# abelxiaoxing/ImageClassification

Measured on AMD Instinct MI355X. Metric: images/sec (whole node) ResNet-50 bf16 224^2 training, higher is better.
Workload: dtype bf16; 1 GPU; resnet50 train step, synthetic 3x224x224, batch 256/GPU, AdamW, label smoothing 0.1, 1000 classes (BASELINE configs[1]); global_batch=256, parallelism=dp1

## Files before the change

imageclassification_amd/csrc/capi.hip:

```cpp
#include "../../include/icamd.h"
#include "common.h"
#include "icamd_internal.h"
#include <cstdlib>
#include <string.h>

int icamd_bn_finalize_launch(const float* part, int nrows, int C, double count, const float* gamma, const float* beta,
                             float* running_mean, float* running_var, float momentum, float eps, float* mean,
                             float* invstd, float* scale, float* shift, double* chunks, hipStream_t s);
int icamd_bn_eval_coeffs_launch(int C, const float* gamma, const float* beta, const float* rm, const float* rv, float eps,
                                float* scale, float* shift, hipStream_t s);
int icamd_bn_apply_launch(const bf16_t* y, const float* scale, const float* shift, const bf16_t* residual, bf16_t* out,
                          unsigned char* maskbits, long long numel, int C, int relu, hipStream_t s,
                          const float* res_scale = nullptr, const float* res_shift = nullptr);
int icamd_bn_bwd_rows_per_block(long long rows, int C);
int icamd_bn_bwd_launch(const bf16_t* dout, const bf16_t* act, const bf16_t* y, const float* mean, const float* invstd,
                        const float* scale, const float* shift, float* dgamma, float* dbeta, bf16_t* dy, bf16_t* gout,
                        const unsigned char* maskbits, long long rows, int C, int relu, int accumulate, float* part,
                        double* chunks, float* c1c2, hipStream_t s, const unsigned char* pool_idx = nullptr,
                        int pool_ih = 0, int pool_iw = 0);
int icamd_bn_bwd_dual_launch(const bf16_t* dout, const unsigned char* maskbits, const bf16_t* yA, const float* meanA,
                             const float* invstdA, const float* scaleA, float* dgammaA, float* dbetaA, bf16_t* dyA,
                             const bf16_t* yB, const float* meanB, const float* invstdB, const float* scaleB, float* dgammaB,
                             float* dbetaB, bf16_t* dyB, long long rows, int C, int accumulate, float* partA, double* chunksA,
                             float* cA, float* partB, double* chunksB, float* cB, hipStream_t s);
// ... 115 lines not shown
  return c;
}
}

namespace {

bool conv_desc_ok(const icamd_conv_desc* d) {
  if (d == nullptr) return false;
  if (d->N <= 0 || d->IH <= 0 || d->IW <= 0 || d->Cin <= 0 || d->OH <= 0 || d->OW <= 0 || d->Cout <= 0) return false;
  if (d->KH <= 0 || d->KW <= 0 || d->stride <= 0 || d->pad < 0) return false;
  if (d->Cin % 64 == 0 && d->KH * d->KW > ICAMD_MAX_TAPS) return false;
  if (d->KH * d->KW > 1024) return false;
  if ((d->IH + 2 * d->pad - d->KH) / d->stride + 1 != d->OH) return false;
  if ((d->IW + 2 * d->pad - d->KW) / d->stride + 1 != d->OW) return false;
  return true;
}

inline size_t align_up(size_t v, size_t a) { return (v + a - 1) / a * a; }

}

extern "C" {

int icamd_abi_version(void) { return 5; }

int icamd_prof_enable(int on) { g_prof_on = on != 0; return ICAMD_OK; }
int icamd_prof_classes(void) { return PC_COUNT; }
int icamd_prof_collect(double* ms, long long* calls, double* bytes, double* flops, int n) {
  if (ms == nullptr || calls == nullptr || n < PC_COUNT) return ICAMD_ERR_BAD_ARG;
  for (auto& r : g_prof_recs) {
    (void)hipEventSynchronize(r.b);
    float t = 0.f;
    (void)hipEventElapsedTime(&t, r.a, r.b);
    ms[r.cls] += (double)t;
    calls[r.cls] += 1;
    if (bytes != nullptr) bytes[r.cls] += r.bytes;
    if (flops != nullptr) flops[r.cls] += r.flops;
    g_prof_pool.push_back(r.a);
    g_prof_pool.push_back(r.b);
  }
  g_prof_recs.clear();
  return ICAMD_OK;
}

int icamd_conv2d_stats_rows(const icamd_conv_desc* d) {
  if (!conv_desc_ok(d)) return 0;
  const long long M = (long long)d->N * d->OH * d->OW;
// ... 218 lines not shown
  return dgrad_impl(d, dy, w_t, dz, nullptr, nullptr, nullptr, stream, z);
}

int icamd_conv2d_dgrad_stats_rows(const icamd_conv_desc* d) {
  if (!conv_desc_ok(d)) return 0;
  int rows = 0;
  for (int ph = 0; ph < d->stride; ++ph)
    for (int pw = 0; pw < d->stride; ++pw) {
      const long long P = (d->IH - ph + d->stride - 1) / d->stride, Q = (d->IW - pw + d->stride - 1) / d->stride;
      if (P > 0 && Q > 0) rows += (int)((d->N * P * Q + 127) / 128);
    }
  return rows;
}

int icamd_conv2d_dgrad_bnbwd(const icamd_conv_desc* d, const void* dy, const void* w_t, void* g, const void* addend,
                             const icamd_bn_bwd_fuse* f, void* stream) {
  ProfScope _prof(PC_IGEMM_DGRAD, stream);
  const ConvWork cw = conv_work(d); _prof.work(cw.out + 2 * cw.in + 2 * cw.w + (addend ? cw.in : 0), cw.flops);
  if (f == nullptr || f->y == nullptr || f->mean == nullptr || f->invstd == nullptr || f->partials == nullptr)
    return ICAMD_ERR_BAD_ARG;
  return dgrad_impl(d, dy, w_t, g, addend, nullptr, f, stream);
}

int icamd_conv2d_dgrad_bnred_supported(const icamd_conv_desc* d) {
  if (!conv_desc_ok(d) || d->KH != 1 || d->KW != 1 || d->stride != 1 || d->pad != 0) return 0;
  return icamd_pw_resident_bnred_wanted((long long)d->N * d->IH * d->IW, d->Cin, d->Cout) ? 1 : 0;
}

int icamd_conv2d_dgrad_bnred(const icamd_conv_desc* d, const void* dy, const void* w_t, void* g, const void* addend,
                             const uint8_t* addend_bits, int addend_sub2, const void* bn_y, const uint8_t* bn_bits,
                             float* partials, void* stream) {
  ProfScope _prof(PC_IGEMM_DGRAD, stream);
  const ConvWork cw = conv_work(d); _prof.work(cw.out + 3 * cw.in + 2 * cw.w + cw.in / 16 + (addend_bits ? cw.in / 16 : 0), cw.flops);
  if (!conv_desc_ok(d) || dy == nullptr || w_t == nullptr || g == nullptr || addend == nullptr || bn_y == nullptr ||
      bn_bits == nullptr || partials == nullptr || (addend_sub2 && addend_bits != nullptr))
    return ICAMD_ERR_BAD_ARG;
  if (!icamd_conv2d_dgrad_bnred_supported(d)) return ICAMD_ERR_UNSUPPORTED;
  PwResidentParams p;
  memset(&p, 0, sizeof(p));
  p.A = (const bf16_t*)dy; p.B = (const bf16_t*)w_t; p.out = (bf16_t*)g; p.addend = (const bf16_t*)addend;
  p.addend_bits = addend_bits;
  p.bn_y = (const bf16_t*)bn_y; p.bn_bits = bn_bits; p.bn_part = partials;
  p.M = d->N * d->IH * d->IW; p.N = d->Cin; p.K = d->Cout;
  if (addend_sub2) { p.sub2_h = d->IH; p.sub2_w = d->IW; }
  return icamd_pw_resident_bnred_launch(p, (hipStream_t)stream);
}
// ... 189 lines not shown
  if (dout == nullptr || maskbits == nullptr || yA == nullptr || yB == nullptr || meanA == nullptr || meanB == nullptr ||
      invstdA == nullptr || invstdB == nullptr || scaleA == nullptr || scaleB == nullptr || dgammaA == nullptr ||
      dgammaB == nullptr || dbetaA == nullptr || dbetaB == nullptr || dyA == nullptr || dyB == nullptr ||
      workspaceA == nullptr || workspaceB == nullptr || workspaceA == workspaceB || rows <= 0 || C <= 0)
    return ICAMD_ERR_BAD_ARG;
  if (workspace_bytes < icamd_bn_bwd_workspace_bytes(rows, C)) return ICAMD_ERR_WORKSPACE;
  if (C > 4096) return ICAMD_ERR_UNSUPPORTED;
  const int rpb = icamd_bn_bwd_rows_per_block(rows, C);
  const long long nblk = (rows + rpb - 1) / rpb;
  float* part[2]; double* chunks[2]; float* cc[2];
  void* wsv[2] = {workspaceA, workspaceB};
  for (int i = 0; i < 2; ++i) {
    char* ws = (char*)wsv[i];
    chunks[i] = (double*)(ws + 256);
    ws += bn_chunk_bytes(C);
    part[i] = (float*)ws;
    ws += align_up((size_t)nblk * 2 * C * sizeof(float), 256);
    cc[i] = (float*)ws;
  }
  return icamd_bn_bwd_dual_launch((const bf16_t*)dout, maskbits, (const bf16_t*)yA, meanA, invstdA, scaleA, dgammaA, dbetaA,
                                  (bf16_t*)dyA, (const bf16_t*)yB, meanB, invstdB, scaleB, dgammaB, dbetaB, (bf16_t*)dyB, rows,
                                  C, accumulate, part[0], chunks[0], cc[0], part[1], chunks[1], cc[1], (hipStream_t)stream);
}

size_t icamd_bn_bwd_apply_workspace_bytes(int C) {
  return C > 0 ? bn_chunk_bytes(C) + align_up((size_t)2 * C * sizeof(float), 256) : 0;
}

int icamd_bn_bwd_from_partials(const float* partials, int nrows, const void* g, const void* y, const float* mean,
                               const float* invstd, const float* scale, float* dgamma, float* dbeta, void* dy,
                               long long rows, int C, int accumulate, void* workspace, size_t workspace_bytes,
                               void* stream) {
  ProfScope _prof(PC_BN_BWD, stream);
  _prof.work((double)rows * C * 6 + 8.0 * nrows * C);
  if (partials == nullptr || nrows <= 0 || g == nullptr || y == nullptr || mean == nullptr || invstd == nullptr ||
      scale == nullptr || dgamma == nullptr || dbeta == nullptr || dy == nullptr || workspace == nullptr || rows <= 0 ||
      C <= 0 || C % 8 != 0)
    return ICAMD_ERR_BAD_ARG;
  if (workspace_bytes < icamd_bn_bwd_apply_workspace_bytes(C)) return ICAMD_ERR_WORKSPACE;
  if (C > 4096) return ICAMD_ERR_UNSUPPORTED;
  char* ws = (char*)workspace;
  double* chunks = (double*)(ws + 256);
  ws += bn_chunk_bytes(C);
  return icamd_bn_bwd_apply_launch(partials, nrows, (const bf16_t*)g, (const bf16_t*)y, mean, invstd, scale, dgamma, dbeta,
                                   (bf16_t*)dy, rows, C, accumulate, chunks, (float*)ws, (hipStream_t)stream);
}
// ... 579 lines not shown
```

imageclassification_amd/csrc/conv3x3_halo.hip:

```cpp
#ifndef ICAMD_C64_NT
#define ICAMD_C64_NT 0
#endif
#include "common.h"
#include "icamd_internal.h"
#include <cstdlib>

namespace {

template <int N> __device__ __forceinline__ void halo_wait_vmcnt() {
  static_assert(N >= 0 && N < 64, "vmcnt is a 6-bit field");
  asm volatile("s_waitcnt vmcnt(%0)" ::"n"(N) : "memory");
}

__device__ __forceinline__ int swzq(int blk) { return (0x78 >> (2 * blk)) & 3; }

template <int BN, int WN, int MFR, int LA, int NB, int KS, int WPS>
__global__ __launch_bounds__(256, WPS) void conv3x3_halo_kernel(const Halo3x3Params p) {
  constexpr int WM = 4 / WN;
  constexpr int BM = WM * MFR * 16;
  constexpr int NJ = BN / WN / 16;
  constexpr int A_SLOTS = 4 * LA * 8;
  constexpr int ZERO_SLOT = A_SLOTS - 1;
  constexpr int A_BYTES = A_SLOTS * 128;
  constexpr int B_STAGE = BN * KS * 2;
// ... 215 lines not shown
  if (p.stats != nullptr) {
    __syncthreads();
    float* red = (float*)smem;
#pragma unroll
    for (int e = 0; e < 8; ++e) {
      red[(rg * 2 + 0) * BN + cp * 8 + e] = s1[e];
      red[(rg * 2 + 1) * BN + cp * 8 + e] = s2[e];
    }
    __syncthreads();
    const int ntm = (p.M + BM - 1) / BM, nrows = (p.M + 127) / 128;
    for (int idx = tid; idx < 2 * BN; idx += 256) {
      const int which = idx / BN, c = idx - which * BN;
      float s = 0.f;
#pragma unroll 4
      for (int g = 0; g < RPP; ++g) s += red[(g * 2 + which) * BN + c];
      if (n0 + c < p.Cout) {
        p.stats[((long long)tile_m * 2 + which) * p.Cout + n0 + c] = s;
        if (ntm + tile_m < nrows) p.stats[((long long)(ntm + tile_m) * 2 + which) * p.Cout + n0 + c] = 0.f;
      }
    }
  }
}

template <bool ACT>
__global__ __launch_bounds__(256, 2) void conv3x3_c64_resident_kernel(const Halo3x3Params p, const int ntiles) {
  constexpr int BM = 128, LA = 8;
  constexpr int A_BYTES = 32 * LA * 128;
  constexpr int E_BYTES = 4 * 64 * 64;
  constexpr int ZERO_SLOT = 32 * LA - 1;
  __shared__ __attribute__((aligned(16))) unsigned char smem[2 * A_BYTES + E_BYTES];

  const int tid = threadIdx.x, lane = tid & 63;
  const int wave = __builtin_amdgcn_readfirstlane(tid >> 6);
  const int wm = wave & 1, wn = wave >> 1;
  const int fr = lane & 15, fq = lane >> 4;
  const int W = p.W, H = p.H;
  const bf16_t* __restrict__ in = p.in;
  const bf16_t* zero = (const bf16_t*)icamd_zero_page;
  unsigned char* const sE = smem + 2 * A_BYTES + wave * 4096;
  const unsigned lds_base = (unsigned)(uintptr_t)LPTR(smem);

  const int a_slot = wave * 8 + (lane >> 3);
  const int a_lc = (((lane & 7) - (lane >> 3)) & 7) * 8;
  const bool a_zero_lane = a_slot == 31;
  auto stage_a = [&](int m0, unsigned char* dst) {
    const int pix0 = m0 - (W + 1) + a_slot;
    const bf16_t* src0 = in + ((long long)pix0 * 64 + a_lc);
// ... 112 lines not shown
    for (int j = 0; j < 2; ++j) {
      f32x4 b4 = {0.f, 0.f, 0.f, 0.f};
      if constexpr (ACT) {
        if (p.bias != nullptr) b4 = *(const f32x4*)(p.bias + wn * 32 + j * 16 + 4 * fq);
      }
#pragma unroll
      for (int i = 0; i < 4; ++i) {
        const int pl = i * 16 + fr;
        f32x4 v = acc[j][i];
        if constexpr (ACT) {
          v += b4;
          if (p.relu) {
#pragma unroll
            for (int e = 0; e < 4; ++e) v[e] = v[e] < 0.f ? 0.f : v[e];
          }
        }
        u32x2 pk;
        pk[0] = pack_bf16x2(v[0], v[1]);
        pk[1] = pack_bf16x2(v[2], v[3]);
        const int slot = j * 4 + fq;
        *(u32x2*)(sE + pl * 64 + ((((slot >> 1) ^ (pl >> 2)) & 3) << 4) + ((slot & 1) << 3)) = pk;
      }
    }
    {
      const int pl0 = lane >> 2;
      const int mrow = m0 + wm * 64 + pl0;
      bf16_t* orow = p.out + ((long long)mrow * 64 + wn * 32 + (lane & 3) * 8);
      const bool want_stats = p.stats != nullptr;
#pragma unroll
      for (int r = 0; r < 4; ++r) {
        const int pl = r * 16 + pl0;
        const u32x4 o = *(const u32x4*)(sE + pl * 64 + ((((lane & 3) ^ (pl >> 2)) & 3) << 4));
        if (mrow + r * 16 < p.M) {
          *(u32x4*)(orow + r * (16 * 64)) = o;
          if (want_stats) {
#pragma unroll
            for (int e = 0; e < 4; ++e) {
              const f32x2 v = {bf16_lo(o[e]), bf16_hi(o[e])};
              s1[e] += v;
              s2[e] = __builtin_elementwise_fma(v, v, s2[e]);
            }
          }
        }
      }
    }
  }

  if (p.stats != nullptr) {
    __syncthreads();
    float* red = (float*)smem;
    const int g = wm * 16 + (lane >> 2);
    const int c0 = wn * 32 + (lane & 3) * 8;
#pragma unroll
    for (int e = 0; e < 4; ++e) {
      red[(g * 2 + 0) * 64 + c0 + 2 * e] = s1[e][0];
      red[(g * 2 + 0) * 64 + c0 + 2 * e + 1] = s1[e][1];
      red[(g * 2 + 1) * 64 + c0 + 2 * e] = s2[e][0];
      red[(g * 2 + 1) * 64 + c0 + 2 * e + 1] = s2[e][1];
    }
    __syncthreads();
    if (tid < 128) {
      const int which = tid >> 6, c = tid & 63;
      float s = 0.f;
#pragma unroll 8
      for (int k = 0; k < 32; ++k) s += red[(k * 2 + which) * 64 + c];
      p.stats[((long long)blockIdx.x * 2 + which) * 64 + c] = s;
      const int nrows = (p.M + 127) / 128;
      for (int r = blockIdx.x + gridDim.x; r < nrows; r += gridDim.x) p.stats[((long long)r * 2 + which) * 64 + c] = 0.f;
    }
  }
}

int launch_resident_c64(const Halo3x3Params& p, hipStream_t stream) {
  const int ntiles = (p.M + 127) / 128;
  const int slots = 2 * icamd_num_cus();
  const int grid = ntiles < slots ? ntiles : slots;
  if (p.bias != nullptr || p.relu)
    hipLaunchKernelGGL((conv3x3_c64_resident_kernel<true>), dim3((unsigned)grid), dim3(256), 0, stream, p, ntiles);
  else
    hipLaunchKernelGGL((conv3x3_c64_resident_kernel<false>), dim3((unsigned)grid), dim3(256), 0, stream, p, ntiles);
  return icamd_launch_status();
}

template <int BN, int WN, int MFR, int LA, int NB, int KS, int WPS>
int launch_halo(const Halo3x3Params& p, hipStream_t stream) {
  constexpr int BM = (4 / WN) * MFR * 16;
  const int ntm = (p.M + BM - 1) / BM;
  hipLaunchKernelGGL((conv3x3_halo_kernel<BN, WN, MFR, LA, NB, KS, WPS>), dim3((unsigned)(ntm * p.ntiles_n)), dim3(256), 0,
                     stream, p);
  return icamd_launch_status();
}

int halo_mode() {
  static const int m = [] { const char* e = getenv("ICAMD_CONV3X3_HALO"); return e ? atoi(e) : 1; }();
  return m;
}

}

static bool resident_c64_ok(int W, int C, int Cout) {
  static const int on = [] { const char* e = getenv("ICAMD_CONV3X3_RESIDENT"); return e ? atoi(e) : 1; }();
  return on != 0 && C == 64 && Cout == 64 && W % 8 == 0 && 128 + 2 * W + 2 <= 255;
}

bool icamd_halo3x3_wanted(int N, int H, int W, int C, int Cout) {
  if (halo_mode() == 0) return false;
  if (C % 64 != 0 || Cout % 8 != 0 || W < 3 || H < 3) return false;
  if (resident_c64_ok(W, C, Cout)) return true;
  if (halo_mode() == 1 && C < 256) return false;
  if ((long long)N * H * W >= (1ll << 30)) return false;
  if (2 * W + 3 + 128 > 4 * 8 * 8) return false;
  return true;
}

int icamd_halo3x3_launch(Halo3x3Params& p, hipStream_t stream) {
  if (!icamd_halo3x3_wanted(p.N, p.H, p.W, p.C, p.Cout)) return ICAMD_ERR_UNSUPPORTED;
  p.M = p.N * p.H * p.W;
  p.divHW = make_fastdiv((unsigned)(p.H * p.W));
  p.divW = make_fastdiv((unsigned)p.W);
  if (resident_c64_ok(p.W, p.C, p.Cout)) return launch_resident_c64(p, stream);
  const int bn = p.Cout <= 64 ? 64 : 128;
  p.ntiles_n = (p.Cout + bn - 1) / bn;
  int bm = 128;
  if (halo_mode() == 3) bm = 256;
  else if (halo_mode() != 2) {
    long long best = -1;
    for (int cand : {256, 224, 128}) {
      if (cand == 224 && bn != 128) continue;
      if ((cand + 2 * p.W + 3 + 31) / 32 > (cand == 128 ? 8 : 12)) continue;
      const long long tiles = (long long)((p.M + cand - 1) / cand) * p.ntiles_n;
      const long long cost = ((tiles + 511) / 512) * cand + (cand == 128 ? 16 : 0);
      if (best < 0 || cost < best) { best = cost; bm = cand; }
    }
  }
  const bool big = bm != 128;
  const int slots = bm + 2 * p.W + 2 + 1;
  const int la = (slots + 31) / 32;
  if (la > 12) return ICAMD_ERR_UNSUPPORTED;
  if (bn == 128) {
// ... 24 lines not shown
```

imageclassification_amd/csrc/icamd_internal.h:

```cpp
#pragma once
#include "common.h"

#define ICAMD_MAX_TAPS 56

struct IgemmParams {
  const bf16_t* in;
  const bf16_t* wt;
  bf16_t* out;
  const bf16_t* addend;
  const unsigned char* addend_bits;
  int addend_sub2;
  const float* bias;
  float* stats;
  const bf16_t* bnb_y;
  const bf16_t* bnb_mask;
  const float *bnb_mean, *bnb_invstd, *bnb_scale, *bnb_shift;
  int bnb_relu;
  int relu;
  bf16_t* gelu_out;
  int gelu_inplace;
  const bf16_t* gelu_z;
  int N, IH, IW, Cin;
  int OH, OW, Cout;
  int P, Q, M;
  int ostr, ooff_h, ooff_w, istr;
  int ntaps, Ktot;
  int KW, pad;
  int tap_sign, regular_taps;
  int stem7;
  int ksteps, ntiles_n;
  FastDiv divPQ, divQ, divCin, divKW;
  short dh[ICAMD_MAX_TAPS], dw[ICAMD_MAX_TAPS], wtap[ICAMD_MAX_TAPS];
};
int icamd_igemm_launch(IgemmParams& p, hipStream_t stream);
int icamd_igemm_pick_bn(int Cout);

struct Halo3x3Params {
  const bf16_t* in;
  const bf16_t* wt;
  bf16_t* out;
  const float* bias;
  float* stats;
  int relu;
  int flip;
  int N, H, W, C, Cout;
  int M, ntiles_n;
  FastDiv divHW, divW;
};
bool icamd_halo3x3_wanted(int N, int H, int W, int C, int Cout);
int icamd_halo3x3_launch(Halo3x3Params& p, hipStream_t stream);

struct GemmNtParams {
  const bf16_t* A;
  const bf16_t* B;
  bf16_t* out;
  const bf16_t* addend;
  const unsigned char* addend_bits;
  const float* bias;
  float* stats;
  int M, N, K;
  int sub2_h, sub2_w;
  FastDiv divHW, divW;
  int relu;
  bf16_t* gelu_out;
  int gelu_inplace;
  const bf16_t* gelu_z;
  int ntiles_n;
  int group_n;
  int out_policy;
};
int icamd_gemm_nt_launch(GemmNtParams& p, hipStream_t stream);
bool icamd_gemm_nt_wanted(long long M, int N, int K);
// ... 108 lines not shown
```

imageclassification_amd/hip.py:

```python
import ctypes
import os
from ctypes import POINTER, Structure, c_double, c_float, c_int, c_longlong, c_size_t, c_void_p

import torch

_HERE = os.path.dirname(os.path.abspath(__file__))
LIB_PATH = os.path.join(_HERE, "csrc", "libicamd.so")

ABI_VERSION = 5
ERRORS = {1: "ICAMD_ERR_BAD_ARG", 2: "ICAMD_ERR_UNSUPPORTED", 3: "ICAMD_ERR_WORKSPACE", 4: "ICAMD_ERR_LAUNCH"}


class IcamdError(RuntimeError):
    pass


class BnBwdFuse(Structure):
    _fields_ = [("y", c_void_p), ("mask_src", c_void_p), ("mean", c_void_p), ("invstd", c_void_p), ("scale", c_void_p),
                ("shift", c_void_p), ("partials", c_void_p), ("relu", c_int)]


class ImageDesc(Structure):
    _fields_ = [("src_offset", ctypes.c_int64), ("src_h", c_int), ("src_w", c_int), ("crop_top", c_int), ("crop_left", c_int),
                ("crop_h", c_int), ("crop_w", c_int), ("hflip", c_int), ("vflip", c_int), ("jitter_order", c_int * 3),
                ("jitter_factor", c_float * 3), ("erase_top", c_int), ("erase_left", c_int), ("erase_h", c_int),
                ("erase_w", c_int), ("erase_seed", ctypes.c_uint32), ("reserved", c_int)]


class ConvDesc(Structure):
    _fields_ = [(n, c_int) for n in ("N", "IH", "IW", "Cin", "OH", "OW", "Cout", "KH", "KW", "stride", "pad")]

    def key(self):
        return tuple(getattr(self, n) for n, _ in self._fields_)


def conv_desc(N, IH, IW, Cin, Cout, KH, KW, stride, pad):
    OH = (IH + 2 * pad - KH) // stride + 1
    OW = (IW + 2 * pad - KW) // stride + 1
    return ConvDesc(N, IH, IW, Cin, OH, OW, Cout, KH, KW, stride, pad)


_P = c_void_p
_SIGNATURES = {
    "icamd_abi_version": (c_int, []),
    "icamd_conv2d_fwd_gelu": (c_int, [_P, _P, _P, _P, _P, _P, _P]),
    "icamd_conv2d_dgrad_gelu": (c_int, [_P, _P, _P, _P, _P, _P]),
    "icamd_conv2d_fwd_act": (c_int, [_P, _P, _P, _P, _P, _P, c_int, _P]),
    "icamd_bn_fold_filters": (c_int, [_P, _P, _P, _P, _P, c_float, c_int, c_int, _P, _P, _P]),
    "icamd_conv2d_stats_rows": (c_int, [POINTER(ConvDesc)]),
    "icamd_conv2d_fwd": (c_int, [POINTER(ConvDesc), _P, _P, _P, _P, _P, _P, _P]),
    "icamd_conv2d_dgrad": (c_int, [POINTER(ConvDesc), _P, _P, _P, _P, _P, _P]),
    "icamd_conv2d_dgrad_sub2": (c_int, [POINTER(ConvDesc), _P, _P, _P, _P, _P]),
    "icamd_conv2d_dgrad_stats_rows": (c_int, [POINTER(ConvDesc)]),
    "icamd_conv2d_dgrad_bnbwd": (c_int, [POINTER(ConvDesc), _P, _P, _P, _P, POINTER(BnBwdFuse), _P]),
    "icamd_conv2d_dgrad_bnred_supported": (c_int, [POINTER(ConvDesc)]),
    "icamd_conv2d_dgrad_bnred": (c_int, [POINTER(ConvDesc), _P, _P, _P, _P, _P, c_int, _P, _P, _P, _P]),
    "icamd_bn_bwd_from_gy_partials": (c_int, [_P, c_int, _P, _P, _P, _P, _P, _P, _P, _P, c_longlong, c_int, c_int, _P, c_size_t, _P]),
    "icamd_bn_apply_conv1x1_fused_supported": (c_int, [POINTER(ConvDesc)]),
    "icamd_bn_apply_conv1x1_fused": (c_int, [POINTER(ConvDesc), _P, _P, _P, _P, _P, _P, _P, _P, _P, _P, _P, _P]),
    "icamd_conv1x1_bn_bwd_fused_supported": (c_int, [POINTER(ConvDesc)]),
    "icamd_conv1x1_bn_bwd_fused_workspace_bytes": (c_size_t, [POINTER(ConvDesc)]),
    "icamd_conv1x1_bn_bwd_fused": (c_int, [POINTER(ConvDesc), _P, c_int, _P, _P, _P, _P, _P, _P, _P, _P, _P, _P, _P, c_int, _P, c_size_t,
                                           _P, c_size_t, _P]),
    "icamd_conv2d_wgrad_workspace_bytes": (c_size_t, [POINTER(ConvDesc)]),
    "icamd_conv2d_wgrad": (c_int, [POINTER(ConvDesc), _P, _P, _P, c_int, _P, c_size_t, _P]),
    "icamd_conv2d_wgrad_bias": (c_int, [POINTER(ConvDesc), _P, _P, _P, _P, c_int, _P, c_size_t, _P]),
    "icamd_filter_transpose": (c_int, [_P, _P, _P, _P, c_int, _P]),
    "icamd_filter_transpose_tiled": (c_int, [_P, _P, _P, _P, c_int, _P]),
    "icamd_bn_workspace_bytes": (c_size_t, [c_int]),
    "icamd_bn_train_finalize": (c_int, [_P, c_int, c_int, c_double, _P, _P, _P, _P, c_float, c_float, _P, _P, _P, _P, _P, _P]),
    "icamd_bn_eval_coeffs": (c_int, [c_int, _P, _P, _P, _P, c_float, _P, _P, _P]),
    "icamd_bn_apply": (c_int, [_P, _P, _P, _P, _P, _P, c_longlong, c_int, c_int, _P]),
    "icamd_bn_apply_res_bn": (c_int, [_P, _P, _P, _P, _P, _P, _P, _P, c_longlong, c_int, c_int, _P]),
    "icamd_bn_bwd_workspace_bytes": (c_size_t, [c_longlong, c_int]),
    "icamd_bn_bwd": (c_int, [_P, _P, _P, _P, _P, _P, _P, _P, _P, _P, _P, _P, c_longlong, c_int, c_int, c_int, _P, c_size_t, _P]),
    "icamd_bn_bwd_maxpool3x3s2": (c_int, [_P, _P, _P, _P, _P, _P, _P, _P, _P, _P, c_int, c_int, c_int, c_int, c_int, _P, c_size_t, _P]),
    "icamd_bn_bwd_dual": (c_int, [_P, _P, _P, _P, _P, _P, _P, _P, _P, _P, _P, _P, _P, _P, _P, _P, c_longlong, c_int, c_int,
# ... 128 lines not shown
```

imageclassification_amd/nets.py:

```python
import ctypes
import math
import os
from collections import OrderedDict

import torch

from . import hip
from .checkpoint import PicklableModel

BN_EPS = 1e-5
_FUSED_BNBWD = os.environ.get("ICAMD_FUSED_BNBWD", "0") == "1"
_WGRAD_STREAM = os.environ.get("ICAMD_WGRAD_STREAM", "1") != "0"
_DUAL_BNBWD = os.environ.get("ICAMD_DUAL_BNBWD", "1") != "0"
_SUB2_SHORTCUT = os.environ.get("ICAMD_SUB2_SHORTCUT", "1") != "0"
_FUSED_POOL_BWD = os.environ.get("ICAMD_FUSED_POOL_BWD", "0") == "1"
BN_MOMENTUM = 0.1

ARCHS = {
    "resnet18": ("basic", [2, 2, 2, 2]),
    "resnet34": ("basic", [3, 4, 6, 3]),
    "resnet50": ("bottleneck", [3, 4, 6, 3]),
}


def _align(n, a):
    return (n + a - 1) // a * a


class _Param:
    __slots__ = ("name", "offset", "numel", "torch_shape", "kind", "padded_shape")

    def __init__(self, name, offset, numel, torch_shape, kind, padded_shape):
        self.name, self.offset, self.numel = name, offset, numel
        self.torch_shape, self.kind, self.padded_shape = torch_shape, kind, padded_shape


class _Conv:
# ... 372 lines not shown
            return ws
        dev = self.device
        lib = self.lib
        ws = {"N": N, "H": H, "W": W}

        def act(n, h, w, c):
            return torch.empty(n, h, w, c, dtype=torch.bfloat16, device=dev)

        Ws = W + (W & 1)
        ws["Ws"] = Ws
        ws["x8"] = act(N, H, Ws + 8, 4)
        d0 = self.stem_conv.desc(N, H, Ws)
        ws["y0"] = act(N, d0.OH, d0.OW, 64)
        ws["a0"] = act(N, d0.OH, d0.OW, 64)
        PH, PW = (d0.OH - 1) // 2 + 1, (d0.OW - 1) // 2 + 1
        ws["p0"] = act(N, PH, PW, 64)
        ws["p0_idx"] = torch.empty(N, PH, PW, 64, dtype=torch.uint8, device=dev)
        max_act = max(ws["y0"].numel(), ws["x8"].numel())
        max_stats = lib.icamd_conv2d_stats_rows(ctypes.byref(d0)) * 2 * 64
        max_wg = lib.icamd_stem7x7s2_wgrad_workspace_bytes(N, H, Ws, 64)
        max_bnb = lib.icamd_bn_bwd_workspace_bytes(N * d0.OH * d0.OW, 64)
        h, w = PH, PW
        blocks_ws = []
        for blk in self.blocks:
            b = {}
            ih, iw = h, w
            ys, acts = [], []
            for ci, conv in enumerate(blk["convs"]):
                d = conv.desc(N, ih, iw)
                ys.append(act(N, d.OH, d.OW, conv.cout_p))
                acts.append(act(N, d.OH, d.OW, conv.cout_p))
                max_act = max(max_act, ys[-1].numel())
                max_stats = max(max_stats, lib.icamd_conv2d_stats_rows(ctypes.byref(d)) * 2 * conv.cout_p)
                max_wg = max(max_wg, lib.icamd_conv2d_wgrad_workspace_bytes(ctypes.byref(d)))
                max_bnb = max(max_bnb, lib.icamd_bn_bwd_workspace_bytes(N * d.OH * d.OW, conv.cout_p))
                ih, iw = d.OH, d.OW
            b["y"], b["a"] = ys, acts
            b["mask"] = torch.empty(acts[-1].numel() // 8, dtype=torch.uint8, device=dev)
            if "down_conv" in blk:
                dd = blk["down_conv"].desc(N, h, w)
                b["yd"] = act(N, dd.OH, dd.OW, blk["down_conv"].cout_p)
                b["ad"] = act(N, dd.OH, dd.OW, blk["down_conv"].cout_p)
                max_stats = max(max_stats, lib.icamd_conv2d_stats_rows(ctypes.byref(dd)) * 2 * blk["down_conv"].cout_p)
                max_wg = max(max_wg, lib.icamd_conv2d_wgrad_workspace_bytes(ctypes.byref(dd)))
                max_bnb = max(max_bnb, lib.icamd_bn_bwd_workspace_bytes(N * dd.OH * dd.OW, blk["down_conv"].cout_p))
            blocks_ws.append(b)
            h, w = ih, iw
        ws["blocks"] = blocks_ws
        ws["final_hw"] = (h, w)
        ws["pooled"] = torch.empty(N, self.feat_dim, dtype=torch.bfloat16, device=dev)
        ws["logits"] = torch.zeros(N, self.ncls_p, dtype=torch.bfloat16, device=dev)
        dfc = self.fc.desc(N, 1, 1)
        max_wg = max(max_wg, lib.icamd_conv2d_wgrad_workspace_bytes(ctypes.byref(dfc)))
        ws["stats"] = torch.empty(max_stats, dtype=torch.float32, device=dev)
        ws["bn_ws"] = torch.zeros(lib.icamd_bn_workspace_bytes(2048), dtype=torch.uint8, device=dev)
        ws["wgrad_ws"] = torch.empty(max_wg, dtype=torch.uint8, device=dev)
        ws["wgrad_ws_bytes"] = max_wg
        ws["bnb_part"] = torch.empty(max_stats + 4 * 2 * 2048, dtype=torch.float32, device=dev)
        ws["bna_ws_bytes"] = lib.icamd_bn_bwd_apply_workspace_bytes(2048)
        ws["bna_ws"] = torch.zeros(ws["bna_ws_bytes"], dtype=torch.uint8, device=dev)
        ws["bnb_ws"] = torch.zeros(max_bnb, dtype=torch.uint8, device=dev)
        ws["bnb_ws2"] = torch.zeros(max_bnb, dtype=torch.uint8, device=dev)
        ws["bnb_ws_bytes"] = max_bnb
        ws["max_act"] = max_act
        ws["loss_rows"] = torch.empty(N, dtype=torch.float32, device=dev)
        ws["pred"] = torch.empty(N, dtype=torch.int32, device=dev)
        ws["dlogits"] = torch.zeros(N, self.ncls_p, dtype=torch.bfloat16, device=dev)
        ws["dpooled"] = torch.empty(N, self.feat_dim, dtype=torch.bfloat16, device=dev)
        ws["scale_shift_eval"] = torch.empty(2 * 2048, dtype=torch.float32, device=dev)
        self._ws[key] = ws
        return ws

    def _grad_buffers(self, ws):
        if "gbuf" not in ws:
            n = ws["max_act"]
            ws["gbuf"] = [torch.empty(n, dtype=torch.bfloat16, device=self.device) for _ in range(8)]
        return ws["gbuf"]

    def _w(self, conv):
        return self.shadow.data_ptr() + 2 * conv.w.offset

# ... 208 lines not shown

        dl = ws["dlogits"].data_ptr()
        wgrad(self.fc, ws["pooled"].data_ptr(), dl, N, 1, 1)
        hip.check(lib.icamd_colsum(dl, N, self.ncls_p, self.ncls_p, self._gf(self.fc.b), acc, s), "fc bias grad")
        dgrad(self.fc, dl, ws["dpooled"].data_ptr(), None, N, 1, 1)
        if hook:
            hook(self.fc.w.offset, self.n_params, side_events())
        fh, fw = ws["final_hw"]
        dout, other = D0, D1
        hip.check(lib.icamd_avgpool_bwd(ws["dpooled"].data_ptr(), dout, N, fh * fw, self.feat_dim, s), "avgpool bwd")

        fused_rows = 0
        for bi in range(len(self.blocks) - 1, -1, -1):
            blk, b = self.blocks[bi], ws["blocks"][bi]
            convs, bns = blk["convs"], blk["bns"]
            h, w = b["in_hw"]
            xin = b["in"]
            nconv = len(convs)
            hw_in = [(h, w)]
            for conv in convs[:-1]:
                d = conv.desc(N, *hw_in[-1])
                hw_in.append((d.OH, d.OW))
            mask = b["mask"].data_ptr()
            yk = next_y()
            y2 = None
            fused_conv3 = False
            shortcut_done = False
            prev_takes_g = False
            if bi > 0 and self.block == "bottleneck":
                pblk = self.blocks[bi - 1]
                if "down_conv" not in pblk:
                    prev_takes_g = True
                else:
                    dp3 = pblk["convs"][-1].desc(N, h, w)
                    prev_takes_g = bool(lib.icamd_conv1x1_bn_bwd_fused_supported(ctypes.byref(dp3)))
            d3 = convs[-1].desc(N, *hw_in[-1])
            fuse3 = (self.block == "bottleneck" and fused_rows > 0
                     and bool(lib.icamd_conv1x1_bn_bwd_fused_supported(ctypes.byref(d3))))

            def fused_conv_bn(conv, bn, dsc, partials, nrows, y_t, x_ptr, dx_ptr, bn_ws, bn_ws_bytes):
                st_ = self.stat_arena.data_ptr() + 4 * bn.stat_offset
                c_ = bn.c
                need = lib.icamd_conv1x1_bn_bwd_fused_workspace_bytes(ctypes.byref(dsc))
                fws = ws.get("fused_ws")
                if fws is None or fws.numel() < need:
                    fws = ws["fused_ws"] = torch.empty(need, dtype=torch.uint8, device=self.device)
                hip.check(lib.icamd_conv1x1_bn_bwd_fused(ctypes.byref(dsc), partials, nrows, dout, y_t.data_ptr(), st_, st_ + 4 * c_,
                                                         st_ + 8 * c_, self._gf(bn.weight), self._gf(bn.bias), x_ptr, self._wt(conv),
                                                         dx_ptr, self._gf(conv.w), acc, bn_ws, bn_ws_bytes, fws.data_ptr(),
                                                         fws.numel(), s), bn.name + " + " + conv.name + " bwd (fused)")

            if "down_conv" in blk and fuse3:
                fused_conv_bn(convs[-1], bns[-1], d3, ws["bnb_part"].data_ptr(), fused_rows, b["y"][-1],
                              b["a"][nconv - 2].data_ptr(), DA, ws["bna_ws"].data_ptr(), ws["bna_ws_bytes"])
                fused_conv3 = True
                dc = blk["down_conv"]
                ddc = dc.desc(N, h, w)
                if dc.stride == 1 and lib.icamd_conv1x1_bn_bwd_fused_supported(ctypes.byref(ddc)):
                    fused_conv_bn(dc, blk["down_bn"], ddc, None, 0, b["yd"], xin.data_ptr(), T, bws, bwb)
                    shortcut_done = True
                else:
                    y2 = next_y()
                    bn_bwd(blk["down_bn"], dout, None, b["yd"], ypool[y2], None, False)
            elif "down_conv" in blk and _DUAL_BNBWD:
                y2 = next_y()
                bnA, bnB = bns[-1], blk["down_bn"]
                stA = self.stat_arena.data_ptr() + 4 * bnA.stat_offset
                stB = self.stat_arena.data_ptr() + 4 * bnB.stat_offset
                c = bnA.c
                hip.check(lib.icamd_bn_bwd_dual(dout, mask, b["y"][-1].data_ptr(), stA, stA + 4 * c, stA + 8 * c,
                                                self._gf(bnA.weight), self._gf(bnA.bias), ypool[yk], b["yd"].data_ptr(), stB,
                                                stB + 4 * c, stB + 8 * c, self._gf(bnB.weight), self._gf(bnB.bias), ypool[y2],
                                                b["y"][-1].numel() // c, c, acc, bws, ws["bnb_ws2"].data_ptr(), bwb, s),
                          bnA.name + " + shortcut bwd")
            elif fused_rows:
                bnl = bns[-1]
                stl = self.stat_arena.data_ptr() + 4 * bnl.stat_offset
                cl = bnl.c
                if fuse3:
                    fused_conv_bn(convs[-1], bnl, d3, ws["bnb_part"].data_ptr(), fused_rows, b["y"][-1],
                                  b["a"][nconv - 2].data_ptr(), DA, ws["bna_ws"].data_ptr(), ws["bna_ws_bytes"])
                    fused_conv3 = True
                else:
                    hip.check(lib.icamd_bn_bwd_from_gy_partials(ws["bnb_part"].data_ptr(), fused_rows, dout, b["y"][-1].data_ptr(),
                                                                stl, stl + 4 * cl, stl + 8 * cl, self._gf(bnl.weight),
                                                                self._gf(bnl.bias), ypool[yk], b["y"][-1].numel() // cl, cl, acc,
                                                                ws["bna_ws"].data_ptr(), ws["bna_ws_bytes"], s),
                              bnl.name + " bwd (apply, sums from the data gradient)")
            else:
                bn_bwd(bns[-1], dout, None, b["y"][-1], ypool[yk], None, True, mask)
            fused_rows = 0
            for i in range(nconv - 1, 0, -1):
                x_i = b["a"][i - 1]
                if fused_conv3 and i == nconv - 1:
                    yk = next_y()
                    bn_bwd(bns[i - 1], DA, None, b["y"][i - 1], ypool[yk], None, True)
                    continue
                wgrad(convs[i], x_i.data_ptr(), ypool[yk], N, *hw_in[i], ybuf=yk)
                dgrad(convs[i], ypool[yk], DA, None, N, *hw_in[i])
                yk = next_y()
                bn_bwd(bns[i - 1], DA, None, b["y"][i - 1], ypool[yk], None, True)
            wgrad(convs[0], xin.data_ptr(), ypool[yk], N, h, w, ybuf=yk)
            if shortcut_done:
                dgrad(convs[0], ypool[yk], other, T, N, h, w)
            elif "down_conv" in blk:
                if y2 is None:
                    y2 = next_y()
                    bn_bwd(blk["down_bn"], dout, None, b["yd"], ypool[y2], None, True, mask)
                dc = blk["down_conv"]
                wgrad(dc, xin.data_ptr(), ypool[y2], N, h, w, ybuf=y2)
                if _SUB2_SHORTCUT and dc.k == 1 and dc.stride == 2 and dc.pad == 0:
                    dd = dc.desc(N, h, w)
                    key = ("sub2", N, dd.OH, dd.OW)
                    d1 = dc.descs.get(key)
                    if d1 is None:
                        d1 = dc.descs[key] = hip.conv_desc(N, dd.OH, dd.OW, dc.cin_p, dc.cout_p, 1, 1, 1, 0)
                    hip.check(lib.icamd_conv2d_dgrad(ctypes.byref(d1), ypool[y2], self._wt(dc), T, None, None, s),
                              dc.name + " dgrad (even grid)")
                    d0 = convs[0].desc(N, h, w)
                    if (prev_takes_g and self.block == "bottleneck"
                            and lib.icamd_conv2d_dgrad_bnred_supported(ctypes.byref(d0))):
# ... 160 lines not shown
```

include/icamd.h:

```cpp
#ifndef ICAMD_H
#define ICAMD_H
#include <stddef.h>
#include <stdint.h>

#ifdef __cplusplus
extern "C" {
#endif

#define ICAMD_OK 0
#define ICAMD_ERR_BAD_ARG 1
#define ICAMD_ERR_UNSUPPORTED 2
#define ICAMD_ERR_WORKSPACE 3
#define ICAMD_ERR_LAUNCH 4

int icamd_abi_version(void);

typedef struct icamd_conv_desc {
  int N, IH, IW, Cin;
  int OH, OW, Cout;
  int KH, KW, stride, pad;
} icamd_conv_desc;

int icamd_conv2d_stats_rows(const icamd_conv_desc* d);

// ... 53 lines not shown
                 const float* scale, const float* shift, float* dgamma, float* dbeta, void* dy, void* gout,
                 const uint8_t* maskbits, long long rows, int C, int relu, int accumulate, void* workspace,
                 size_t workspace_bytes, void* stream);
int icamd_bn_bwd_maxpool3x3s2(const void* dout_pooled, const uint8_t* idx, const void* y, const float* mean,
                              const float* invstd, const float* scale, const float* shift, float* dgamma, float* dbeta,
                              void* dy, int N, int IH, int IW, int C, int accumulate, void* workspace, size_t workspace_bytes,
                              void* stream);

int icamd_bn_bwd_dual(const void* dout, const uint8_t* maskbits, const void* yA, const float* meanA, const float* invstdA,
                      const float* scaleA, float* dgammaA, float* dbetaA, void* dyA, const void* yB, const float* meanB,
                      const float* invstdB, const float* scaleB, float* dgammaB, float* dbetaB, void* dyB, long long rows, int C,
                      int accumulate, void* workspaceA, void* workspaceB, size_t workspace_bytes, void* stream);

size_t icamd_bn_bwd_apply_workspace_bytes(int C);
int icamd_bn_bwd_from_partials(const float* partials, int nrows, const void* g, const void* y, const float* mean,
                               const float* invstd, const float* scale, float* dgamma, float* dbeta, void* dy,
                               long long rows, int C, int accumulate, void* workspace, size_t workspace_bytes,
                               void* stream);

int icamd_conv2d_dgrad_bnred_supported(const icamd_conv_desc* d);
int icamd_conv2d_dgrad_bnred(const icamd_conv_desc* d, const void* dy, const void* w_t, void* g, const void* addend,
                             const uint8_t* addend_bits, int addend_sub2, const void* bn_y, const uint8_t* bn_bits,
                             float* partials, void* stream);
int icamd_bn_bwd_from_gy_partials(const float* partials, int nrows, const void* g, const void* y, const float* mean,
                                  const float* invstd, const float* scale, float* dgamma, float* dbeta, void* dy,
                                  long long rows, int C, int accumulate, void* workspace, size_t workspace_bytes,
                                  void* stream);

int icamd_bn_apply_conv1x1_fused_supported(const icamd_conv_desc* d);
int icamd_bn_apply_conv1x1_fused(const icamd_conv_desc* d, const void* y, const float* scale, const float* shift,
                                 const void* residual, const float* res_scale, const float* res_shift, void* out,
                                 uint8_t* maskbits, const void* w, void* y1, float* stats, void* stream);

int icamd_conv1x1_bn_bwd_fused_supported(const icamd_conv_desc* d);
size_t icamd_conv1x1_bn_bwd_fused_workspace_bytes(const icamd_conv_desc* d);
int icamd_conv1x1_bn_bwd_fused(const icamd_conv_desc* d, const float* partials, int nrows, const void* g, const void* y,
                               const float* mean, const float* invstd, const float* scale, float* dgamma, float* dbeta,
                               const void* x, const void* w_t, void* dx, float* dw, int accumulate, void* bn_workspace,
                               size_t bn_workspace_bytes, void* wgrad_workspace, size_t wgrad_workspace_bytes, void* stream);

int icamd_layernorm_fwd(const void* x, const float* gamma, const float* beta, void* y, float* mean, float* rstd,
                        long long rows, int C, float eps, void* stream);
size_t icamd_layernorm_bwd_workspace_bytes(long long rows, int C);
int icamd_layernorm_bwd(const void* dy, const void* x, const float* mean, const float* rstd, const float* gamma,
                        const void* addend, void* dx, float* dgamma, float* dbeta, long long rows, int C, int accumulate,
                        void* workspace, size_t workspace_bytes, void* stream);
// ... 120 lines not shown
```

Measured before the change: 14240 images/sec.

## Fuse ReLU mask and BN-backward reductions into 3x3 halo dgrad epilogue

Adds a BN-reduce variant of the resident 3x3 c64 halo conv kernel for dgrad. It recomputes the ReLU mask from the saved BN input and scale/shift, writes the masked gradient, and accumulates per-channel sum(g) and sum(g*y) partials in the epilogue. The inner bottleneck BN backward then only runs the apply pass from those partials, so one full read of the gradient tensor is no longer needed. It also preallocates the fused 1x1 workspace instead of growing it inside the loop. The cost is extra loads of y and the scale/shift vectors plus more register pressure in the conv epilogue, and it applies only to 64-channel 3x3 stride-1 layers.

New measurement: 14230 images/sec (median of 3 runs). About the same (-0.1%).

```diff
diff --git a/imageclassification_amd/csrc/capi.hip b/imageclassification_amd/csrc/capi.hip
--- a/imageclassification_amd/csrc/capi.hip
+++ b/imageclassification_amd/csrc/capi.hip
@@ -161,7 +161,7 @@
 
 extern "C" {
 
-int icamd_abi_version(void) { return 5; }
+int icamd_abi_version(void) { return 6; }
 
 int icamd_prof_enable(int on) { g_prof_on = on != 0; return ICAMD_OK; }
 int icamd_prof_classes(void) { return PC_COUNT; }
@@ -426,6 +426,36 @@
   return dgrad_impl(d, dy, w_t, g, addend, nullptr, f, stream);
 }
 
+int icamd_conv2d_dgrad_bnred_relu_supported(const icamd_conv_desc* d) {
+  if (!conv_desc_ok(d) || d->KH != 3 || d->KW != 3 || d->stride != 1 || d->pad != 1) return 0;
+  if ((long long)d->N * d->IH * d->IW >= (1ll << 31)) return 0;
+  return icamd_halo3x3_bnred_wanted(d->N, d->IH, d->IW, d->Cout, d->Cin) ? 1 : 0;
+}
+
+int icamd_conv2d_dgrad_bnred_relu_rows(const icamd_conv_desc* d) {
+  if (!icamd_conv2d_dgrad_bnred_relu_supported(d)) return 0;
+  return (int)(((long long)d->N * d->IH * d->IW + 127) / 128);
+}
+
+int icamd_conv2d_dgrad_bnred_relu(const icamd_conv_desc* d, const void* dy, const void* w_t, void* g, const void* bn_y,
+                                  const float* bn_scale, const float* bn_shift, float* partials, void* stream) {
+  ProfScope _prof(PC_IGEMM_DGRAD, stream);
+  if (d != nullptr) {
+    const ConvWork cw = conv_work(d);
+    _prof.work(cw.out + 2 * cw.in + 2 * cw.w + 8.0 * icamd_conv2d_dgrad_bnred_relu_rows(d) * d->Cin, cw.flops);
+  }
+  if (!conv_desc_ok(d) || dy == nullptr || w_t == nullptr || g == nullptr || bn_y == nullptr || bn_scale == nullptr ||
+      bn_shift == nullptr || partials == nullptr)
+    return ICAMD_ERR_BAD_ARG;
+  if (!icamd_conv2d_dgrad_bnred_relu_supported(d)) return ICAMD_ERR_UNSUPPORTED;
+  Halo3x3Params h;
+  memset(&h, 0, sizeof(h));
+  h.in = (const bf16_t*)dy; h.wt = (const bf16_t*)w_t; h.out = (bf16_t*)g; h.flip = 1;
+  h.N = d->N; h.H = d->IH; h.W = d->IW; h.C = d->Cout; h.Cout = d->Cin;
+  h.stats = partials; h.bn_y = (const bf16_t*)bn_y; h.bn_scale = bn_scale; h.bn_shift = bn_shift;
+  return icamd_halo3x3_launch(h, (hipStream_t)stream);
+}
+
 int icamd_conv2d_dgrad_bnred_supported(const icamd_conv_desc* d) {
   if (!conv_desc_ok(d) || d->KH != 1 || d->KW != 1 || d->stride != 1 || d->pad != 0) return 0;
   return icamd_pw_resident_bnred_wanted((long long)d->N * d->IH * d->IW, d->Cin, d->Cout) ? 1 : 0;
@@ -661,6 +691,7 @@
                                   (bf16_t*)dyA, (const bf16_t*)yB, meanB, invstdB, scaleB, dgammaB, dbetaB, (bf16_t*)dyB, rows,
                                   C, accumulate, part[0], chunks[0], cc[0], part[1], chunks[1], cc[1], (hipStream_t)stream);
 }
+
 
 size_t icamd_bn_bwd_apply_workspace_bytes(int C) {
   return C > 0 ? bn_chunk_bytes(C) + align_up((size_t)2 * C * sizeof(float), 256) : 0;
diff --git a/imageclassification_amd/csrc/conv3x3_halo.hip b/imageclassification_amd/csrc/conv3x3_halo.hip
--- a/imageclassification_amd/csrc/conv3x3_halo.hip
+++ b/imageclassification_amd/csrc/conv3x3_halo.hip
@@ -261,7 +261,7 @@
   }
 }
 
-template <bool ACT>
+template <bool ACT, bool BNR = false>
 __global__ __launch_bounds__(256, 2) void conv3x3_c64_resident_kernel(const Halo3x3Params p, const int ntiles) {
   constexpr int BM = 128, LA = 8;
   constexpr int A_BYTES = 32 * LA * 128;
@@ -420,7 +420,7 @@
         *(u32x2*)(sE + pl * 64 + ((((slot >> 1) ^ (pl >> 2)) & 3) << 4) + ((slot & 1) << 3)) = pk;
       }
     }
-    {
+    if constexpr (!BNR) {
       const int pl0 = lane >> 2;
       const int mrow = m0 + wm * 64 + pl0;
       bf16_t* orow = p.out + ((long long)mrow * 64 + wn * 32 + (lane & 3) * 8);
@@ -438,6 +438,45 @@
               s1[e] += v;
               s2[e] = __builtin_elementwise_fma(v, v, s2[e]);
             }
+          }
+        }
+      }
+    } else {
+      const int pl0 = lane >> 2;
+      const int mrow = m0 + wm * 64 + pl0;
+      int c0 = wn * 32 + (lane & 3) * 8;
+      asm volatile("" : "+v"(c0));
+      bf16_t* orow = p.out + ((long long)mrow * 64 + c0);
+      u32x4 yv[4];
+#pragma unroll
+      for (int r = 0; r < 4; ++r)
+        yv[r] = *(const u32x4*)(mrow + r * 16 < p.M ? p.bn_y + ((long long)(mrow + r * 16) * 64 + c0) : zero);
+      f32x4 gsc[2], gsh[2];
+#pragma unroll
+      for (int h = 0; h < 2; ++h) {
+        gsc[h] = *(const f32x4*)(p.bn_scale + c0 + 4 * h);
+        gsh[h] = *(const f32x4*)(p.bn_shift + c0 + 4 * h);
+      }
+      asm volatile("" : "+v"(gsc[0]), "+v"(gsc[1]), "+v"(gsh[0]), "+v"(gsh[1]));
+#pragma unroll
+      for (int r = 0; r < 4; ++r) {
+        const int pl = r * 16 + pl0;
+        u32x4 o = *(const u32x4*)(sE + pl * 64 + ((((lane & 3) ^ (pl >> 2)) & 3) << 4));
+        if (mrow + r * 16 < p.M) {
+          f32x2 yy[4];
+#pragma unroll
+          for (int e = 0; e < 4; ++e) {
+            yy[e] = f32x2{bf16_lo(yv[r][e]), bf16_hi(yv[r][e])};
+            const bool klo = fmaf(yy[e][0], gsc[e >> 1][(2 * e) & 3], gsh[e >> 1][(2 * e) & 3]) > 0.f;
+            const bool khi = fmaf(yy[e][1], gsc[e >> 1][(2 * e + 1) & 3], gsh[e >> 1][(2 * e + 1) & 3]) > 0.f;
+            o[e] &= (klo ? 0x0000FFFFu : 0u) | (khi ? 0xFFFF0000u : 0u);
+          }
+          *(u32x4*)(orow + r * (16 * 64)) = o;
+#pragma unroll
+          for (int e = 0; e < 4; ++e) {
+            const f32x2 v = {bf16_lo(o[e]), bf16_hi(o[e])};
+            s1[e] += v;
+            s2[e] = __builtin_elementwise_fma(v, yy[e], s2[e]);
           }
         }
       }
@@ -473,7 +512,9 @@
   const int ntiles = (p.M + 127) / 128;
   const int slots = 2 * icamd_num_cus();
   const int grid = ntiles < slots ? ntiles : slots;
-  if (p.bias != nullptr || p.relu)
+  if (p.bn_y != nullptr)
+    hipLaunchKernelGGL((conv3x3_c64_resident_kernel<false, true>), dim3((unsigned)grid), dim3(256), 0, stream, p, ntiles);
+  else if (p.bias != nullptr || p.relu)
     hipLaunchKernelGGL((conv3x3_c64_resident_kernel<true>), dim3((unsigned)grid), dim3(256), 0, stream, p, ntiles);
   else
     hipLaunchKernelGGL((conv3x3_c64_resident_kernel<false>), dim3((unsigned)grid), dim3(256), 0, stream, p, ntiles);
@@ -511,8 +552,15 @@
   return true;
 }
 
+bool icamd_halo3x3_bnred_wanted(int N, int H, int W, int C, int Cout) {
+  return icamd_halo3x3_wanted(N, H, W, C, Cout) && resident_c64_ok(W, C, Cout);
+}
+
 int icamd_halo3x3_launch(Halo3x3Params& p, hipStream_t stream) {
   if (!icamd_halo3x3_wanted(p.N, p.H, p.W, p.C, p.Cout)) return ICAMD_ERR_UNSUPPORTED;
+  if (p.bn_y != nullptr && (p.bias != nullptr || p.relu || p.stats == nullptr || p.bn_scale == nullptr || p.bn_shift == nullptr ||
+                            !resident_c64_ok(p.W, p.C, p.Cout)))
+    return ICAMD_ERR_UNSUPPORTED;
   p.M = p.N * p.H * p.W;
   p.divHW = make_fastdiv((unsigned)(p.H * p.W));
   p.divW = make_fastdiv((unsigned)p.W);
diff --git a/imageclassification_amd/csrc/icamd_internal.h b/imageclassification_amd/csrc/icamd_internal.h
--- a/imageclassification_amd/csrc/icamd_internal.h
+++ b/imageclassification_amd/csrc/icamd_internal.h
@@ -46,8 +46,11 @@
   int N, H, W, C, Cout;
   int M, ntiles_n;
   FastDiv divHW, divW;
+  const bf16_t* bn_y;
+  const float *bn_scale, *bn_shift;
 };
 bool icamd_halo3x3_wanted(int N, int H, int W, int C, int Cout);
+bool icamd_halo3x3_bnred_wanted(int N, int H, int W, int C, int Cout);
 int icamd_halo3x3_launch(Halo3x3Params& p, hipStream_t stream);
 
 struct GemmNtParams {
diff --git a/imageclassification_amd/hip.py b/imageclassification_amd/hip.py
--- a/imageclassification_amd/hip.py
+++ b/imageclassification_amd/hip.py
@@ -7,7 +7,7 @@
 _HERE = os.path.dirname(os.path.abspath(__file__))
 LIB_PATH = os.path.join(_HERE, "csrc", "libicamd.so")
 
-ABI_VERSION = 5
+ABI_VERSION = 6
 ERRORS = {1: "ICAMD_ERR_BAD_ARG", 2: "ICAMD_ERR_UNSUPPORTED", 3: "ICAMD_ERR_WORKSPACE", 4: "ICAMD_ERR_LAUNCH"}
 
 
@@ -53,6 +53,9 @@
     "icamd_conv2d_dgrad_sub2": (c_int, [POINTER(ConvDesc), _P, _P, _P, _P, _P]),
     "icamd_conv2d_dgrad_stats_rows": (c_int, [POINTER(ConvDesc)]),
     "icamd_conv2d_dgrad_bnbwd": (c_int, [POINTER(ConvDesc), _P, _P, _P, _P, POINTER(BnBwdFuse), _P]),
+    "icamd_conv2d_dgrad_bnred_relu_supported": (c_int, [POINTER(ConvDesc)]),
+    "icamd_conv2d_dgrad_bnred_relu_rows": (c_int, [POINTER(ConvDesc)]),
+    "icamd_conv2d_dgrad_bnred_relu": (c_int, [POINTER(ConvDesc), _P, _P, _P, _P, _P, _P, _P, _P]),
     "icamd_conv2d_dgrad_bnred_supported": (c_int, [POINTER(ConvDesc)]),
     "icamd_conv2d_dgrad_bnred": (c_int, [POINTER(ConvDesc), _P, _P, _P, _P, _P, c_int, _P, _P, _P, _P]),
     "icamd_bn_bwd_from_gy_partials": (c_int, [_P, c_int, _P, _P, _P, _P, _P, _P, _P, _P, c_longlong, c_int, c_int, _P, c_size_t, _P]),
diff --git a/imageclassification_amd/nets.py b/imageclassification_amd/nets.py
--- a/imageclassification_amd/nets.py
+++ b/imageclassification_amd/nets.py
@@ -13,6 +13,7 @@
 _WGRAD_STREAM = os.environ.get("ICAMD_WGRAD_STREAM", "1") != "0"
 _DUAL_BNBWD = os.environ.get("ICAMD_DUAL_BNBWD", "1") != "0"
 _SUB2_SHORTCUT = os.environ.get("ICAMD_SUB2_SHORTCUT", "1") != "0"
+_BNRED_INNER = os.environ.get("ICAMD_BNRED_INNER", "1") != "0"
 _FUSED_POOL_BWD = os.environ.get("ICAMD_FUSED_POOL_BWD", "0") == "1"
 BN_MOMENTUM = 0.1
 
@@ -431,8 +432,10 @@
         max_bnb = lib.icamd_bn_bwd_workspace_bytes(N * d0.OH * d0.OW, 64)
         h, w = PH, PW
         blocks_ws = []
+        blocks_hw = []
         for blk in self.blocks:
             b = {}
+            blocks_hw.append((h, w))
             ih, iw = h, w
             ys, acts = [], []
             for ci, conv in enumerate(blk["convs"]):
@@ -466,6 +469,20 @@
         ws["wgrad_ws"] = torch.empty(max_wg, dtype=torch.uint8, device=dev)
         ws["wgrad_ws_bytes"] = max_wg
         ws["bnb_part"] = torch.empty(max_stats + 4 * 2 * 2048, dtype=torch.float32, device=dev)
+        ws["bnb_part_inner"] = torch.empty(max_stats, dtype=torch.float32, device=dev)
+        fused_need = 0
+        for blk, (h, w) in zip(self.blocks, blocks_hw):
+            if self.block != "bottleneck":
+                break
+            hw = (h, w)
+            for conv in blk["convs"][:-1]:
+                d = conv.desc(N, *hw)
+                hw = (d.OH, d.OW)
+            fused_need = max(fused_need, lib.icamd_conv1x1_bn_bwd_fused_workspace_bytes(ctypes.byref(blk["convs"][-1].desc(N, *hw))))
+            if "down_conv" in blk:
+                fused_need = max(fused_need,
+                                 lib.icamd_conv1x1_bn_bwd_fused_workspace_bytes(ctypes.byref(blk["down_conv"].desc(N, h, w))))
+        ws["fused_ws"] = torch.empty(max(fused_need, 1), dtype=torch.uint8, device=dev)
         ws["bna_ws_bytes"] = lib.icamd_bn_bwd_apply_workspace_bytes(2048)
         ws["bna_ws"] = torch.zeros(ws["bna_ws_bytes"], dtype=torch.uint8, device=dev)
         ws["bnb_ws"] = torch.zeros(max_bnb, dtype=torch.uint8, device=dev)
@@ -720,7 +737,7 @@
                 d = conv.desc(N, *hw_in[-1])
                 hw_in.append((d.OH, d.OW))
             mask = b["mask"].data_ptr()
-            yk = next_y()
+            yk = None
             y2 = None
             fused_conv3 = False
             shortcut_done = False
@@ -739,10 +756,7 @@
             def fused_conv_bn(conv, bn, dsc, partials, nrows, y_t, x_ptr, dx_ptr, bn_ws, bn_ws_bytes):
                 st_ = self.stat_arena.data_ptr() + 4 * bn.stat_offset
                 c_ = bn.c
-                need = lib.icamd_conv1x1_bn_bwd_fused_workspace_bytes(ctypes.byref(dsc))
-                fws = ws.get("fused_ws")
-                if fws is None or fws.numel() < need:
-                    fws = ws["fused_ws"] = torch.empty(need, dtype=torch.uint8, device=self.device)
+                fws = ws["fused_ws"]
                 hip.check(lib.icamd_conv1x1_bn_bwd_fused(ctypes.byref(dsc), partials, nrows, dout, y_t.data_ptr(), st_, st_ + 4 * c_,
                                                          st_ + 8 * c_, self._gf(bn.weight), self._gf(bn.bias), x_ptr, self._wt(conv),
                                                          dx_ptr, self._gf(conv.w), acc, bn_ws, bn_ws_bytes, fws.data_ptr(),
@@ -761,6 +775,7 @@
                     y2 = next_y()
                     bn_bwd(blk["down_bn"], dout, None, b["yd"], ypool[y2], None, False)
             elif "down_conv" in blk and _DUAL_BNBWD:
+                yk = next_y()
                 y2 = next_y()
                 bnA, bnB = bns[-1], blk["down_bn"]
                 stA = self.stat_arena.data_ptr() + 4 * bnA.stat_offset
@@ -780,12 +795,14 @@
                                   b["a"][nconv - 2].data_ptr(), DA, ws["bna_ws"].data_ptr(), ws["bna_ws_bytes"])
                     fused_conv3 = True
                 else:
+                    yk = next_y()
                     hip.check(lib.icamd_bn_bwd_from_gy_partials(ws["bnb_part"].data_ptr(), fused_rows, dout, b["y"][-1].data_ptr(),
                                                                 stl, stl + 4 * cl, stl + 8 * cl, self._gf(bnl.weight),
                                                                 self._gf(bnl.bias), ypool[yk], b["y"][-1].numel() // cl, cl, acc,
                                                                 ws["bna_ws"].data_ptr(), ws["bna_ws_bytes"], s),
                               bnl.name + " bwd (apply, sums from the data gradient)")
             else:
+                yk = next_y()
                 bn_bwd(bns[-1], dout, None, b["y"][-1], ypool[yk], None, True, mask)
             fused_rows = 0
             for i in range(nconv - 1, 0, -1):
@@ -795,6 +812,22 @@
                     bn_bwd(bns[i - 1], DA, None, b["y"][i - 1], ypool[yk], None, True)
                     continue
                 wgrad(convs[i], x_i.data_ptr(), ypool[yk], N, *hw_in[i], ybuf=yk)
+                di = convs[i].desc(N, *hw_in[i])
+                if _BNRED_INNER and lib.icamd_conv2d_dgrad_bnred_relu_supported(ctypes.byref(di)):
+                    bn = bns[i - 1]
+                    st = self.stat_arena.data_ptr() + 4 * bn.stat_offset
+                    c = bn.c
+                    part = ws["bnb_part_inner"].data_ptr()
+                    hip.check(lib.icamd_conv2d_dgrad_bnred_relu(ctypes.byref(di), ypool[yk], self._wt(convs[i]), DA,
+                                                                b["y"][i - 1].data_ptr(), st + 8 * c, st + 12 * c, part, s),
+                              convs[i].name + " dgrad + bn reduce")
+                    yk = next_y()
+                    hip.check(lib.icamd_bn_bwd_from_gy_partials(part, lib.icamd_conv2d_dgrad_bnred_relu_rows(ctypes.byref(di)), DA,
+                                                                b["y"][i - 1].data_ptr(), st, st + 4 * c, st + 8 * c,
+                                                                self._gf(bn.weight), self._gf(bn.bias), ypool[yk],
+                                                                b["y"][i - 1].numel() // c, c, acc, ws["bna_ws"].data_ptr(),
+                                                                ws["bna_ws_bytes"], s), bn.name + " bwd (apply, sums from the data gradient)")
+                    continue
                 dgrad(convs[i], ypool[yk], DA, None, N, *hw_in[i])
                 yk = next_y()
                 bn_bwd(bns[i - 1], DA, None, b["y"][i - 1], ypool[yk], None, True)
diff --git a/include/icamd.h b/include/icamd.h
--- a/include/icamd.h
+++ b/include/icamd.h
@@ -99,6 +99,10 @@
 int icamd_conv2d_dgrad_bnred(const icamd_conv_desc* d, const void* dy, const void* w_t, void* g, const void* addend,
                              const uint8_t* addend_bits, int addend_sub2, const void* bn_y, const uint8_t* bn_bits,
                              float* partials, void* stream);
+int icamd_conv2d_dgrad_bnred_relu_supported(const icamd_conv_desc* d);
+int icamd_conv2d_dgrad_bnred_relu_rows(const icamd_conv_desc* d);
+int icamd_conv2d_dgrad_bnred_relu(const icamd_conv_desc* d, const void* dy, const void* w_t, void* g, const void* bn_y,
+                                  const float* bn_scale, const float* bn_shift, float* partials, void* stream);
 int icamd_bn_bwd_from_gy_partials(const float* partials, int nrows, const void* g, const void* y, const float* mean,
                                   const float* invstd, const float* scale, float* dgamma, float* dbeta, void* dy,
                                   long long rows, int C, int accumulate, void* workspace, size_t workspace_bytes,
```
